# robot-perception-group/AirPose

Hardware: AMD Instinct MI355X
Metric: two-view frames/sec at batch 256 (224x224) (higher is better)
Workload: dtype f16; 1 GPU; copenet_twoview forward (ResNet-50 x2 views, 3 IEF iterations) + SMPL-X LBS tail (10475 verts, 127 joints, projection); pairs_per_gpu=256, global_pairs=256, image=224x224, ief_iters=3, trunk_chunk_images=512, trunk_passes=2 concurrent passes (one per view) on 2 HIP streams

## Files before the change

### airpose_amd/csrc/conv_lean.hip

```cpp
#include "ap_common.h"
#include "kernels.h"

AP_NS_BEGIN

namespace {

constexpr int BM = 128, BN = 128, NT = 512, FM = 4, FN = 2, WAVES_N = 4;
constexpr int SLOTS = 3, TILE_BYTES = 16384, A_BYTES = 8192;
constexpr int HALF = 64, CLD = HALF + 4;
constexpr int LDS_BYTES = SLOTS * TILE_BYTES;
static_assert(BM * CLD * 4 <= LDS_BYTES, "the epilogue stage reuses the ring");
constexpr int POOL_IMGS = 5, POOL_PIX = 49, POOL_ROWS = POOL_IMGS * POOL_PIX;
constexpr int PSUM_OFF = BM * CLD * 4, PSUM_BYTES = 3 * 8 * HALF * 4;
constexpr int CARRY_BYTES = 2 * 8 * HALF * 4;
static_assert(PSUM_OFF + PSUM_BYTES <= LDS_BYTES, "partial sums fit behind the stage");
static_assert(3 * (LDS_BYTES + CARRY_BYTES) <= 160 * 1024, "three workgroups per CU");

template <int N> __device__ __forceinline__ void wait_vmcnt() { asm volatile("s_waitcnt vmcnt(%0)" ::"n"(N) : "memory"); }
template <int N> __device__ __forceinline__ void wait_lgkmcnt() {
    asm volatile("s_waitcnt lgkmcnt(%0)" ::"n"(N) : "memory");
    __builtin_amdgcn_sched_barrier(0);
}
template <int OFF> __device__ __forceinline__ u32x4 lds_read_b128(uint32_t addr) {
    u32x4 r;
    asm volatile("ds_read_b128 %0, %1 offset:%2" : "=v"(r) : "v"(addr), "n"(OFF));
    return r;
}
__device__ __forceinline__ void mfma_acc(f32x4& c, const u32x4& w, const u32x4& x) {
    asm volatile(AP_MFMA16_ASM " %0, %1, %2, %0" : "+v"(c) : "v"(w), "v"(x));
}

template <bool POOL>
__global__ void __launch_bounds__(NT) __attribute__((amdgpu_waves_per_eu(6, 6))) conv_lean_kernel(const ConvArgs p) {
    typedef bf16_t T;
    extern __shared__ __attribute__((aligned(1024))) unsigned char smem[];
    const int wave = __builtin_amdgcn_readfirstlane(threadIdx.x >> 6);
    const int wm = wave / WAVES_N, wn = wave % WAVES_N;
    const int tile = xcd_remap(blockIdx.x, p.mtiles * p.ntiles);
    const int bm = tile / p.ntiles, bn = tile % p.ntiles;
    const int KT = p.Cin / 32;
    const unsigned char* zg = (const unsigned char*)p.zero;
    const unsigned char* xg = (const unsigned char*)p.x;
    const unsigned char* wg = (const unsigned char*)p.w;
    asm volatile("" ::"s"(zg), "s"(xg), "s"(wg));

    constexpr int NSUB = POOL ? 2 : 1;
    const int row0 = POOL ? bm * POOL_ROWS : bm * BM;
    const uint32_t lds0 = (uint32_t)(size_t)(__attribute__((address_space(3))) unsigned char*)smem;
    for (int sub = 0; sub < NSUB; ++sub) {
    if (POOL && sub) __syncthreads();
    int tid = threadIdx.x;
    asm volatile("" : "+v"(tid));
    const int lane = tid & 63;
    const int prow = lane >> 2;
    const int pchunk = (lane & 3) ^ ((0x1230 >> ((prow >> 2) * 4)) & 3);
    const int rl_dma = sub * BM + wave * 16 + prow, m = row0 + rl_dma;
    const bool a_ok = m < p.M && (!POOL || rl_dma < POOL_ROWS);
    uint32_t aoff = a_ok ? (uint32_t)(((size_t)m * p.ldx + pchunk * 8) * sizeof(T)) : 0u;
    uint32_t woff = (uint32_t)(((size_t)(bn * BN + wave * 16 + prow) * p.wld + pchunk * 8) * sizeof(T));
    auto issue_tile = [&](int slot) {
        const unsigned char* as = a_ok ? xg + aoff : zg;
        __builtin_amdgcn_global_load_lds((const __attribute__((address_space(1))) void*)as,
                                         (__attribute__((address_space(3))) void*)(smem + slot * TILE_BYTES + wave * 1024), 16, 0, 0);
        __builtin_amdgcn_global_load_lds((const __attribute__((address_space(1))) void*)(wg + woff),
                                         (__attribute__((address_space(3))) void*)(smem + slot * TILE_BYTES + A_BYTES + wave * 1024),
                                         16, 0, 0);
        aoff += 64u; woff += 64u;
        asm volatile("" : "+v"(aoff), "+v"(woff));
    };

    const int lr = lane & 15, g4 = lane >> 4;
    const uint32_t fslot = (uint32_t)(lr * 4 + (g4 ^ ((0x1230 >> ((lr >> 2) * 4)) & 3))) * 16u;
    const uint32_t xa = lds0 + wm * 4096 + fslot;
    const uint32_t wa = lds0 + A_BYTES + wn * 2048 + fslot;
    f32x4 acc[FM][FN];
#pragma unroll
    for (int fm = 0; fm < FM; ++fm)
#pragma unroll
        for (int fn = 0; fn < FN; ++fn) acc[fm][fn] = f32x4{0.f, 0.f, 0.f, 0.f};

    issue_tile(0);
    if (KT > 1) issue_tile(1);
    if (KT > 1) wait_vmcnt<2>();
    else wait_vmcnt<0>();
    __builtin_amdgcn_s_barrier();
    int slot = 0;
    for (int k = 0; k < KT; ++k) {
        const uint32_t so = slot * TILE_BYTES;
        u32x4 xf[FM], wf[FN];
        xf[0] = lds_read_b128<0>(xa + so);
        xf[1] = lds_read_b128<1024>(xa + so);
        xf[2] = lds_read_b128<2048>(xa + so);
        xf[3] = lds_read_b128<3072>(xa + so);
        wf[0] = lds_read_b128<0>(wa + so);
        wf[1] = lds_read_b128<1024>(wa + so);
        if (k + 2 < KT) issue_tile(slot == 0 ? 2 : slot - 1);
        __builtin_amdgcn_sched_barrier(0);
        wait_lgkmcnt<0>();
#pragma unroll
        for (int fm = 0; fm < FM; ++fm)
#pragma unroll
            for (int fn = 0; fn < FN; ++fn) mfma_acc(acc[fm][fn], wf[fn], xf[fm]);
        if (k + 1 < KT) {
            if (k + 2 < KT) wait_vmcnt<2>();
            else wait_vmcnt<0>();
            __builtin_amdgcn_s_barrier();
        }
        slot = slot == 2 ? 0 : slot + 1;
    }
    asm volatile("s_nop 15\n\ts_nop 15" ::: "memory");

    float* ct = (float*)smem;
    T* __restrict__ yg = (T*)p.y;
    const T* __restrict__ rg = (const T*)p.res;
    constexpr int CPR = HALF / 8, NIT = BM * CPR / NT;
    uint32_t rng = 0u;
#pragma unroll
    for (int h = 0; h < 2; ++h) {
        __syncthreads();
        if ((wn >> 1) == h) {
#pragma unroll
            for (int fn = 0; fn < FN; ++fn) {
                const int chl = (wn & 1) * 32 + fn * 16 + g4 * 4;
                const int ch = bn * BN + h * HALF + chl;
                const float4 sc = *(const float4*)(p.scale + ch);
                const float4 sh = *(const float4*)(p.shift + ch);
#pragma unroll
                for (int fm = 0; fm < FM; ++fm) {
                    const int px = wm * 64 + fm * 16 + lr;
                    float4 v;
                    v.x = acc[fm][fn][0] * sc.x + sh.x;
                    v.y = acc[fm][fn][1] * sc.y + sh.y;
                    v.z = acc[fm][fn][2] * sc.z + sh.z;
                    v.w = acc[fm][fn][3] * sc.w + sh.w;
                    *(float4*)(ct + px * CLD + chl) = v;
                }
            }
        }
        __syncthreads();
        u32x4 rv[NIT];
        if (rg) {
#pragma unroll
            for (int it = 0; it < NIT; ++it) {
                const int q = tid + it * NT, px = q / CPR, cc = q - px * CPR;
                const int rl = sub * BM + px, mm = row0 + rl, ch = bn * BN + h * HALF + cc * 8;
                const bool ok = mm < p.M && ch < p.Cout && (!POOL || rl < POOL_ROWS);
                rv[it] = *(const u32x4*)(ok ? rg + (size_t)mm * p.ldr + ch : (const T*)p.zero);
            }
        }
#pragma unroll
        for (int it = 0; it < NIT; ++it) {
            const int q = tid + it * NT, px = q / CPR, cc = q - px * CPR;
            const int rl = sub * BM + px, mm = row0 + rl, ch = bn * BN + h * HALF + cc * 8;
            if (!POOL && (mm >= p.M || ch >= p.Cout)) continue;
            float* sp = ct + px * CLD + cc * 8;
            float4 a = *(const float4*)sp, b = *(const float4*)(sp + 4);
            if (rg) {
                float lo, hi;
#ifdef AP_F16
                (void)lo; (void)hi;
                ap_res_add2(a.x, a.y, rv[it][0]); ap_res_add2(a.z, a.w, rv[it][1]);
                ap_res_add2(b.x, b.y, rv[it][2]); ap_res_add2(b.z, b.w, rv[it][3]);
#else
                unpack_bf16x2(rv[it][0], lo, hi); a.x += lo; a.y += hi;
                unpack_bf16x2(rv[it][1], lo, hi); a.z += lo; a.w += hi;
                unpack_bf16x2(rv[it][2], lo, hi); b.x += lo; b.y += hi;
                unpack_bf16x2(rv[it][3], lo, hi); b.z += lo; b.w += hi;
#endif
            }
            if (p.relu) {
                a.x = ap_relu(a.x); a.y = ap_relu(a.y); a.z = ap_relu(a.z); a.w = ap_relu(a.w);
                b.x = ap_relu(b.x); b.y = ap_relu(b.y); b.z = ap_relu(b.z); b.w = ap_relu(b.w);
            }
            u32x4 o;
            o[0] = pack_bf16x2(a.x, a.y); o[1] = pack_bf16x2(a.z, a.w);
            o[2] = pack_bf16x2(b.x, b.y); o[3] = pack_bf16x2(b.z, b.w);
            ap_rng_note4(rng, o[0], o[1], o[2], o[3], p.relu != 0);
            if constexpr (!POOL) {
                *(u32x4*)(yg + (size_t)mm * p.ldy + ch) = o;
            } else {
                unpack_bf16x2(o[0], a.x, a.y); unpack_bf16x2(o[1], a.z, a.w);
                unpack_bf16x2(o[2], b.x, b.y); unpack_bf16x2(o[3], b.z, b.w);
                *(float4*)sp = a; *(float4*)(sp + 4) = b;
            }
        }
        if constexpr (POOL) {
            __syncthreads();
            float* psum = (float*)(smem + PSUM_OFF);
            float* carry = (float*)(smem + LDS_BYTES) + h * 8 * HALF;
            const int k = tid >> 6, c = tid & 63;
#pragma unroll
            for (int seg = 0; seg < 3; ++seg) {
                const int r0 = sub == 0 ? seg * POOL_PIX : (seg == 0 ? 0 : 19 + (seg - 1) * POOL_PIX);
                const int p0 = (sub == 1 && seg == 0) ? 30 : 0;
                const int p1 = (sub == 0 && seg == 2) ? 30 : POOL_PIX;
                float sacc = (sub == 1 && seg == 0) ? carry[k * HALF + c] : 0.f;
                int px0 = k + ((p0 - k + 7) & ~7);
                if (p0 == 0) px0 = k;
                for (int px = px0; px < p1; px += 8) sacc += ct[(r0 + px - p0) * CLD + c];
                if (sub == 0 && seg == 2) carry[k * HALF + c] = sacc;
                else psum[(seg * 8 + k) * HALF + c] = sacc;
            }
            __syncthreads();
            if (tid < 3 * HALF) {
                const int seg = tid >> 6;
                const int img_l = sub == 0 ? seg : seg + 2;
                const int img = bm * POOL_IMGS + img_l, ch = bn * BN + h * HALF + c;
                if (!(sub == 0 && seg == 2) && img < p.N && ch < p.Cout) {
                    float t = psum[(seg * 8) * HALF + c];
#pragma unroll
                    for (int kk = 1; kk < 8; ++kk) t += psum[(seg * 8 + kk) * HALF + c];
                    p.pool_out[(size_t)img * p.Cout + ch] = t / 49.0f;
                }
            }
        }
    }
    ap_rng_flush(p.range_flag, rng);
    }
}

}

bool ap_conv_lean_supported(const ConvArgs& a, int kind) {
    return kind == K_BF16 && a.KH == 1 && a.KW == 1 && a.stride == 1 && a.pad == 0 && !a.x2 && a.Cin % 32 == 0 && a.Cin >= 32 &&
           (long long)a.M * a.ldx * 2 < 0xffffffffll && (long long)a.wld * 2 * ((a.Cout + 127) / 128 * 128) < 0xffffffffll;
}

hipError_t ap_launch_conv_lean(ConvArgs a, hipStream_t st) {
    if (!a.zero || !ap_conv_lean_supported(a, K_BF16)) return hipErrorInvalidValue;
    a.ntiles = (a.Cout + BN - 1) / BN;
    if (a.pool_out) {
        if (a.Ho * a.Wo != POOL_PIX || a.M != a.N * POOL_PIX || !a.res || !a.relu) return hipErrorInvalidValue;
        static bool attr_set[AP_MAX_DEVICES] = {};
        int dev = 0;
        hipError_t e = ap_current_device(&dev);
        if (e != hipSuccess) return e;
        if (!attr_set[dev]) {
            e = hipFuncSetAttribute((const void*)conv_lean_kernel<true>, hipFuncAttributeMaxDynamicSharedMemorySize, LDS_BYTES + CARRY_BYTES);
            if (e != hipSuccess) return e;
            attr_set[dev] = true;
        }
        a.mtiles = (a.N + POOL_IMGS - 1) / POOL_IMGS;
        hipLaunchKernelGGL(conv_lean_kernel<true>, dim3(a.mtiles * a.ntiles), dim3(NT), LDS_BYTES + CARRY_BYTES, st, a);
        return hipGetLastError();
    }
    a.mtiles = (a.M + BM - 1) / BM;
    hipLaunchKernelGGL(conv_lean_kernel<false>, dim3(a.mtiles * a.ntiles), dim3(NT), LDS_BYTES, st, a);
    return hipGetLastError();
}

AP_NS_END
```

Measured before the change: 49130 pairs/s.

## Make lean 1x1 conv persistent with prefetched residuals and LDS-staged scale/shift

The non-pool 1x1 conv kernel becomes persistent. The grid is capped at three workgroups per CU, and each workgroup walks a contiguous range of tiles assigned to its XCD. The residual tile for the next half or next tile is loaded with nontemporal loads during the current epilogue, so that latency hides behind compute. Per-channel scale and shift are now DMA'd into extra LDS instead of being read from global memory in the epilogue. This adds LDS, register pressure from the held residual vectors, and a barrier between tiles.

Result: no change. 48940 pairs/s (-0.4%).

```diff
diff --git a/airpose_amd/csrc/conv_lean.hip b/airpose_amd/csrc/conv_lean.hip
--- a/airpose_amd/csrc/conv_lean.hip
+++ b/airpose_amd/csrc/conv_lean.hip
@@ -14,7 +14,8 @@
 constexpr int PSUM_OFF = BM * CLD * 4, PSUM_BYTES = 3 * 8 * HALF * 4;
 constexpr int CARRY_BYTES = 2 * 8 * HALF * 4;
 static_assert(PSUM_OFF + PSUM_BYTES <= LDS_BYTES, "partial sums fit behind the stage");
-static_assert(3 * (LDS_BYTES + CARRY_BYTES) <= 160 * 1024, "three workgroups per CU");
+constexpr int SS_BYTES = 2 * BN * 4;
+static_assert(3 * (LDS_BYTES + CARRY_BYTES) <= 160 * 1024 && 3 * (LDS_BYTES + SS_BYTES) <= 160 * 1024, "three workgroups per CU");
 
 template <int N> __device__ __forceinline__ void wait_vmcnt() { asm volatile("s_waitcnt vmcnt(%0)" ::"n"(N) : "memory"); }
 template <int N> __device__ __forceinline__ void wait_lgkmcnt() {
@@ -36,8 +37,10 @@
     extern __shared__ __attribute__((aligned(1024))) unsigned char smem[];
     const int wave = __builtin_amdgcn_readfirstlane(threadIdx.x >> 6);
     const int wm = wave / WAVES_N, wn = wave % WAVES_N;
-    const int tile = xcd_remap(blockIdx.x, p.mtiles * p.ntiles);
-    const int bm = tile / p.ntiles, bn = tile % p.ntiles;
+    const int ntot = p.mtiles * p.ntiles, xcd = blockIdx.x & 7, wi = blockIdx.x >> 3;
+    const int tq = ntot >> 3, tr = ntot & 7;
+    const int t0 = xcd < tr ? xcd * (tq + 1) : tr * (tq + 1) + (xcd - tr) * tq, tcnt = tq + (xcd < tr ? 1 : 0);
+    const int wx = ((int)gridDim.x - xcd + 7) >> 3;
     const int KT = p.Cin / 32;
     const unsigned char* zg = (const unsigned char*)p.zero;
     const unsigned char* xg = (const unsigned char*)p.x;
@@ -45,8 +48,30 @@
     asm volatile("" ::"s"(zg), "s"(xg), "s"(wg));
 
     constexpr int NSUB = POOL ? 2 : 1;
+    constexpr int CPR = HALF / 8, NIT = BM * CPR / NT;
+    const uint32_t lds0 = (uint32_t)(size_t)(__attribute__((address_space(3))) unsigned char*)smem;
+    T* __restrict__ yg = (T*)p.y;
+    const T* __restrict__ rg = (const T*)p.res;
+    uint32_t rng = 0u;
+    u32x4 rvp[NIT];
+    auto res_issue = [&](u32x4 (&rv)[NIT], int tbm, int tbn, int h) __attribute__((always_inline)) {
+        int t = threadIdx.x;
+        asm volatile("" : "+v"(t) : : "memory");
+#pragma unroll
+        for (int it = 0; it < NIT; ++it) {
+            const int q = t + it * NT, px = q / CPR, cc = q - px * CPR;
+            const int mm = tbm * BM + px, ch = tbn * BN + h * HALF + cc * 8;
+            const bool ok = mm < p.M && ch < p.Cout;
+            rv[it] = __builtin_nontemporal_load((const u32x4*)(ok ? rg + (size_t)mm * p.ldr + ch : (const T*)p.zero));
+        }
+        asm volatile("" ::: "memory");
+    };
+    int tl = wi;
+    do {
+    const int tile = t0 + tl;
+    const int bm = tile / p.ntiles, bn = tile % p.ntiles;
     const int row0 = POOL ? bm * POOL_ROWS : bm * BM;
-    const uint32_t lds0 = (uint32_t)(size_t)(__attribute__((address_space(3))) unsigned char*)smem;
+    if (!POOL && rg && tl == wi) res_issue(rvp, bm, bn, 0);
     for (int sub = 0; sub < NSUB; ++sub) {
     if (POOL && sub) __syncthreads();
     int tid = threadIdx.x;
@@ -69,6 +94,11 @@
         asm volatile("" : "+v"(aoff), "+v"(woff));
     };
 
+    if (!POOL && wave < 4) {
+        const float* sr = (wave < 2 ? p.scale : p.shift) + bn * BN + (wave & 1) * 64 + lane;
+        __builtin_amdgcn_global_load_lds((const __attribute__((address_space(1))) void*)sr,
+                                         (__attribute__((address_space(3))) void*)(smem + LDS_BYTES + wave * 256), 4, 0, 0);
+    }
     const int lr = lane & 15, g4 = lane >> 4;
     const uint32_t fslot = (uint32_t)(lr * 4 + (g4 ^ ((0x1230 >> ((lr >> 2) * 4)) & 3))) * 16u;
     const uint32_t xa = lds0 + wm * 4096 + fslot;
@@ -111,10 +141,6 @@
     asm volatile("s_nop 15\n\ts_nop 15" ::: "memory");
 
     float* ct = (float*)smem;
-    T* __restrict__ yg = (T*)p.y;
-    const T* __restrict__ rg = (const T*)p.res;
-    constexpr int CPR = HALF / 8, NIT = BM * CPR / NT;
-    uint32_t rng = 0u;
 #pragma unroll
     for (int h = 0; h < 2; ++h) {
         __syncthreads();
@@ -122,9 +148,16 @@
 #pragma unroll
             for (int fn = 0; fn < FN; ++fn) {
                 const int chl = (wn & 1) * 32 + fn * 16 + g4 * 4;
-                const int ch = bn * BN + h * HALF + chl;
-                const float4 sc = *(const float4*)(p.scale + ch);
-                const float4 sh = *(const float4*)(p.shift + ch);
+                float4 sc, sh;
+                if constexpr (POOL) {
+                    const int ch = bn * BN + h * HALF + chl;
+                    sc = *(const float4*)(p.scale + ch);
+                    sh = *(const float4*)(p.shift + ch);
+                } else {
+                    const float* ss = (const float*)(smem + LDS_BYTES);
+                    sc = *(const float4*)(ss + h * HALF + chl);
+                    sh = *(const float4*)(ss + BN + h * HALF + chl);
+                }
 #pragma unroll
                 for (int fm = 0; fm < FM; ++fm) {
                     const int px = wm * 64 + fm * 16 + lr;
@@ -139,7 +172,10 @@
         }
         __syncthreads();
         u32x4 rv[NIT];
-        if (rg) {
+        if constexpr (!POOL) {
+#pragma unroll
+            for (int it = 0; it < NIT; ++it) rv[it] = rvp[it];
+        } else if (rg) {
 #pragma unroll
             for (int it = 0; it < NIT; ++it) {
                 const int q = tid + it * NT, px = q / CPR, cc = q - px * CPR;
@@ -184,6 +220,10 @@
                 *(float4*)sp = a; *(float4*)(sp + 4) = b;
             }
         }
+        if constexpr (!POOL) {
+            if (rg && h == 0) res_issue(rvp, bm, bn, 1);
+            if (rg && h == 1 && tl + wx < tcnt) res_issue(rvp, (tile + wx) / p.ntiles, (tile + wx) % p.ntiles, 0);
+        }
         if constexpr (POOL) {
             __syncthreads();
             float* psum = (float*)(smem + PSUM_OFF);
@@ -215,8 +255,11 @@
             }
         }
     }
+    }
+    if (POOL || (tl += wx) >= tcnt) break;
+    __syncthreads();
+    } while (true);
     ap_rng_flush(p.range_flag, rng);
-    }
 }
 
 }
@@ -245,7 +288,22 @@
         return hipGetLastError();
     }
     a.mtiles = (a.M + BM - 1) / BM;
-    hipLaunchKernelGGL(conv_lean_kernel<false>, dim3(a.mtiles * a.ntiles), dim3(NT), LDS_BYTES, st, a);
+    static int cus[AP_MAX_DEVICES] = {};
+    int dev = 0;
+    hipError_t e = ap_current_device(&dev);
+    if (e != hipSuccess) return e;
+    if (!cus[dev]) {
+        e = hipDeviceGetAttribute(&cus[dev], hipDeviceAttributeMultiprocessorCount, dev);
+        if (e != hipSuccess) return e;
+    }
+    static bool attr_plain[AP_MAX_DEVICES] = {};
+    if (!attr_plain[dev]) {
+        e = hipFuncSetAttribute((const void*)conv_lean_kernel<false>, hipFuncAttributeMaxDynamicSharedMemorySize, LDS_BYTES + SS_BYTES);
+        if (e != hipSuccess) return e;
+        attr_plain[dev] = true;
+    }
+    const int ntot = a.mtiles * a.ntiles, grid = ntot < 3 * cus[dev] ? ntot : 3 * cus[dev];
+    hipLaunchKernelGGL(conv_lean_kernel<false>, dim3(grid), dim3(NT), LDS_BYTES + SS_BYTES, st, a);
     return hipGetLastError();
 }
 
```
